# BaeHann/feature_level_style_transfer_for_TSC

Hardware: AMD Instinct MI355X
Metric: train-step samples/sec (univariate TS, len=512, batch=256) at 1/2/4/8 MI355X (higher is better)
Workload: dtype bf16x3

## Files before the change

### feature_level_style_transfer_for_tsc_amd/csrc/pointwise.hip

```cpp
#include "fst_common.h"

static thread_local char g_err[512] = "";
void fst_set_error(const char* fmt, ...) {
  va_list ap;
  va_start(ap, fmt);
  vsnprintf(g_err, sizeof(g_err), fmt, ap);
  va_end(ap);
}
extern "C" const char* fst_last_error(void) { return g_err; }

int fst_allow_full_lds(const void* fn, const char* who) {
  static const void* done[64];
  static int n_done = 0;
  for (int i = 0; i < n_done; ++i)
    if (done[i] == fn) return 0;
  hipError_t e = hipFuncSetAttribute(fn, hipFuncAttributeMaxDynamicSharedMemorySize, 160 * 1024);
  if (e != hipSuccess) {
    fst_set_error("%s: hipFuncSetAttribute: %s", who, hipGetErrorString(e));
    return (int)e;
  }
  if (n_done < 64) done[n_done++] = fn;
  return 0;
}
int fst_cu_count(void) {
  static int cached[16] = {0};
  int dev = 0;
  if (hipGetDevice(&dev) != hipSuccess || dev < 0 || dev >= 16) return 0;
  if (cached[dev] == 0) {
    int n = 0;
    if (hipDeviceGetAttribute(&n, hipDeviceAttributeMultiprocessorCount, dev) != hipSuccess) n = 0;
    cached[dev] = n > 0 ? n : -1;
  }
  return cached[dev] > 0 ? cached[dev] : 0;
}
extern "C" int fst_version(void) { return FST_ABI_VERSION; }

__device__ __forceinline__ float wave_sum(float v) {
#pragma unroll
  for (int o = 32; o > 0; o >>= 1) v += __shfl_down(v, o, 64);
  return v;
}

__device__ __forceinline__ void block_sum2(float& a, float& b) {
  __shared__ float sa[4], sb[4];
  a = wave_sum(a);
  b = wave_sum(b);
  const int lane = threadIdx.x & 63, wave = threadIdx.x >> 6;
  if (lane == 0) { sa[wave] = a; sb[wave] = b; }
  __syncthreads();
  if (threadIdx.x == 0) {
    a = sa[0] + sa[1] + sa[2] + sa[3];
    b = sb[0] + sb[1] + sb[2] + sb[3];
  }
  __syncthreads();
}

#define FST_REQUIRE_EXTENT(who, B, C, L, numel)                                                             \
  FST_REQUIRE((long long)(B) * (long long)(C) * (long long)(L) == (long long)(numel),                        \
              "%s: B*C*L = %d*%d*%d does not match the tensors' element count %lld", who, (int)(B), (int)(C), (int)(L), \
              (long long)(numel))


struct RowVec {
  int shift;
  int nv;
};
static inline bool vec_ok(int L, std::initializer_list<const void*> ptrs) {
  if (L % 4 != 0) return false;
  for (const void* q : ptrs)
    if (!fst_aligned16(q)) return false;
  return true;
}
static inline RowVec row_vec(int L) {
  RowVec v;
  v.nv = L / 4;
  v.shift = 0;
  while ((1 << v.shift) < v.nv && v.shift < 8) ++v.shift;
  return v;
}
static inline RowVec row_dword(int L, int shift) { return RowVec{shift, L}; }
constexpr int BN_DWORD_SHIFT = 8, ROW_SUM_DWORD_SHIFT = 6;

template <class V>
__device__ __forceinline__ RowVec row_geometry(RowVec rv, int dword_shift) {
  if (std::is_same_v<V, float>) rv.shift = dword_shift;
  return rv;
}
template <class V>
__device__ __forceinline__ int row_group(RowVec rv, int T) {
  const int r = threadIdx.x >> rv.shift;
  return std::is_same_v<V, float> ? r & ((T >> rv.shift) - 1) : r;
}

template <class Launch>
static inline void launch_rows(bool vec, int L, int dword_shift, Launch launch) {
  if (vec) launch(float4{}, row_vec(L));
  else launch(float{}, row_dword(L, dword_shift));
}

__device__ __forceinline__ float block_sum1024(float s) {
  __shared__ float sw[16];
  s = wave_sum(s);
  const int lane = threadIdx.x & 63, wave = threadIdx.x >> 6;
  if (lane == 0) sw[wave] = s;
  __syncthreads();
  float r = 0.f;
  if (threadIdx.x == 0) {
#pragma unroll
    for (int w = 0; w < 16; ++w) r += sw[w];
  }
  return r;
}

__device__ __forceinline__ void row_sum_add(float& s0, float& s1, const float4& v) {
  s0 += v.x + v.y;
  s1 += v.z + v.w;
}
__device__ __forceinline__ void row_sum_add(float& s0, float&, float v) { s0 += v; }

template <class V>
__global__ __launch_bounds__(1024) void row_sum_kernel(const float* x, long long x_bs, int B, int C, int L, float* out, RowVec rv) {
  rv = row_geometry<V>(rv, ROW_SUM_DWORD_SHIFT);
  const int c = blockIdx.x, r = row_group<V>(rv, 1024), t0 = threadIdx.x & ((1 << rv.shift) - 1), rpp = 1024 >> rv.shift;
  float s0 = 0.f, s1 = 0.f;
  for (int b = r; b < B; b += rpp) {
    const V* row = reinterpret_cast<const V*>(x + (long long)b * x_bs + (long long)c * L);
    for (int t = t0; t < rv.nv; t += 1 << rv.shift) {
      const V v = row[t];
      row_sum_add(s0, s1, v);
    }
  }
  const float s = block_sum1024(std::is_same_v<V, float> ? s0 : s0 + s1);
  if (threadIdx.x == 0) out[c] = s;
}

extern "C" int fst_row_sum(const float* x, int64_t x_bs, int B, int C, int L, float* out, void* stream) {
  FST_REQUIRE(x && out && B > 0 && C > 0 && L > 0, "fst_row_sum: bad arguments");
  FST_REQUIRE(B == 1 || x_bs >= (int64_t)C * L, "fst_row_sum: batch stride %lld < C*L = %lld", (long long)x_bs, (long long)C * L);
  launch_rows(vec_ok(L, {x}) && x_bs % 4 == 0, L, ROW_SUM_DWORD_SHIFT, [&](auto v, RowVec rv) {
    hipLaunchKernelGGL(row_sum_kernel<decltype(v)>, dim3(C), dim3(1024), 0, (hipStream_t)stream, x, (long long)x_bs, B, C, L, out, rv);
  });
  FST_LAUNCH_CHECK();
  return 0;
}

__device__ __forceinline__ void bn_moments_add(float& s1, float& s2, float v, float k) {
  const float d = v - k;
  s1 += d; s2 += d * d;
}
__device__ __forceinline__ void bn_moments_add(float& s1, float& s2, float4 v, float k) {
  const float dx = v.x - k, dy = v.y - k, dz = v.z - k, dw = v.w - k;
  s1 += (dx + dy) + (dz + dw);
  s2 += (dx * dx + dy * dy) + (dz * dz + dw * dw);
}

template <class V>
__global__ __launch_bounds__(256) void bn_stats_kernel(const float* y, int B, int C, int L, float* part, RowVec rv) {
  rv = row_geometry<V>(rv, BN_DWORD_SHIFT);
  const int c = blockIdx.x, r = row_group<V>(rv, 256), t0 = threadIdx.x & ((1 << rv.shift) - 1), rpp = 256 >> rv.shift;
  const float k = y[(long long)c * L];
  float s1 = 0.f, s2 = 0.f;
  for (int b = blockIdx.y + r * gridDim.y; b < B; b += rpp * gridDim.y) {
    const V* row = reinterpret_cast<const V*>(y + ((long long)b * C + c) * L);
    for (int t = t0; t < rv.nv; t += 1 << rv.shift) bn_moments_add(s1, s2, row[t], k);
  }
  block_sum2(s1, s2);
  if (threadIdx.x == 0) {
    const int rows = blockIdx.y < B ? (B - 1 - blockIdx.y) / gridDim.y + 1 : 0;
    float* o = part + ((long long)c * FST_BN_SLOTS + blockIdx.y) * 4;
    o[0] = (float)rows * (float)L; o[1] = k; o[2] = s1; o[3] = s2;
  }
}

extern "C" int fst_bn_stats(const float* y, int B, int C, int L, float* part, int64_t numel, void* stream) {
  FST_REQUIRE(y && part && B > 0 && C > 0 && L > 0, "fst_bn_stats: bad arguments");
  FST_REQUIRE_EXTENT("fst_bn_stats", B, C, L, numel);
  launch_rows(vec_ok(L, {y}), L, BN_DWORD_SHIFT, [&](auto v, RowVec rv) {
    hipLaunchKernelGGL(bn_stats_kernel<decltype(v)>, dim3(C, FST_BN_SLOTS), dim3(256), 0, (hipStream_t)stream, y, B, C, L, part, rv);
  });
  FST_LAUNCH_CHECK();
  return 0;
}

__global__ void bn_finalize_kernel(const float* part, int n_slots, const float* gamma, const float* beta, float* rmean,
                                   float* rvar, int train, int C, float eps, float momentum, float* stats) {
  const int c = blockIdx.x * blockDim.x + threadIdx.x;
  if (c >= C) return;
  float mean, var;
  if (train) {
    double n = 0.0, m = 0.0, m2 = 0.0;
    const float* q = part + (long long)c * n_slots * 4;
    for (int s = 0; s < n_slots; ++s) {
      const double nb = q[4 * s];
      if (nb <= 0.0) continue;
      const double s1 = q[4 * s + 2], s2 = q[4 * s + 3];
      const double mb = (double)q[4 * s + 1] + s1 / nb;
      double Mb = s2 - s1 * s1 / nb;
      if (Mb < 0.0) Mb = 0.0;
      const double nn = n + nb, d = mb - m;
      m += d * (nb / nn);
      m2 += Mb + d * d * (n * nb / nn);
      n = nn;
    }
    const double v = n > 0.0 ? m2 / n : 0.0;
    mean = (float)m;
    var = (float)v;
    const float unbiased = n > 1.0 ? (float)(m2 / (n - 1.0)) : var;
    rmean[c] = (1.f - momentum) * rmean[c] + momentum * mean;
    rvar[c] = (1.f - momentum) * rvar[c] + momentum * unbiased;
  } else {
    mean = rmean[c];
    var = rvar[c];
  }
  const float invstd = 1.0f / sqrtf(var + eps);
  const float scale = gamma[c] * invstd;
  stats[c] = mean;
  stats[C + c] = invstd;
  stats[2 * C + c] = scale;
  stats[3 * C + c] = beta[c] - mean * scale;
}

extern "C" int fst_bn_finalize(const float* part, int n_slots, const float* gamma, const float* beta, float* running_mean,
                               float* running_var, int train, int C, float eps, float momentum, float* stats, void* stream) {
  FST_REQUIRE(gamma && beta && running_mean && running_var && stats && C > 0, "fst_bn_finalize: bad arguments");
  FST_REQUIRE(!train || (part && n_slots > 0), "fst_bn_finalize: train mode needs the moment partials (n_slots=%d)", n_slots);
  hipLaunchKernelGGL(bn_finalize_kernel, dim3((C + 63) / 64), dim3(64), 0, (hipStream_t)stream, part, n_slots, gamma, beta,
                     running_mean, running_var, train, C, eps, momentum, stats);
  FST_LAUNCH_CHECK();
  return 0;
}

__device__ __forceinline__ float bn_pre(float y, float sc, float sh) { return __builtin_fmaf(y, sc, sh); }
__device__ __forceinline__ float bn_pre_join(float ya, float sca, float sha, float yb, float scb, float shb) {
#pragma clang fp contract(off)
  float v = bn_pre(ya, sca, sha);
  v += bn_pre(yb, scb, shb);
  return v;
}
__device__ __forceinline__ float4 bn_pre(float4 y, float sc, float sh) {
  return make_float4(bn_pre(y.x, sc, sh), bn_pre(y.y, sc, sh), bn_pre(y.z, sc, sh), bn_pre(y.w, sc, sh));
}
__device__ __forceinline__ float4 bn_pre_join(float4 ya, float sca, float sha, float4 yb, float scb, float shb) {
  return make_float4(bn_pre_join(ya.x, sca, sha, yb.x, scb, shb), bn_pre_join(ya.y, sca, sha, yb.y, scb, shb),
                     bn_pre_join(ya.z, sca, sha, yb.z, scb, shb), bn_pre_join(ya.w, sca, sha, yb.w, scb, shb));
}
__device__ __forceinline__ float bn_relu(float v) { return v < 0.f ? 0.f : v; }
__device__ __forceinline__ float4 bn_relu(float4 v) { return make_float4(bn_relu(v.x), bn_relu(v.y), bn_relu(v.z), bn_relu(v.w)); }

template <class V>
__global__ __launch_bounds__(256) void bn_apply_kernel(const float* y, const float* stats, const float* res,
                                                       const float* res_stats, float* out, int rows, int C, int L,
                                                       int relu, RowVec rv) {
  rv = row_geometry<V>(rv, BN_DWORD_SHIFT);
  const int r = row_group<V>(rv, 256), t0 = threadIdx.x & ((1 << rv.shift) - 1), rpp = 256 >> rv.shift;
  const int bc = blockIdx.x * rpp + r;
  if (bc >= rows) return;
  const int c = bc % C;
  const float sc = stats[2 * C + c], sh = stats[3 * C + c];
  float rsc = 1.f, rsh = 0.f;
  if (res && res_stats) { rsc = res_stats[2 * C + c]; rsh = res_stats[3 * C + c]; }
  const long long base = (long long)bc * rv.nv;
  const V* yv = reinterpret_cast<const V*>(y) + base;
  const V* qv = res ? reinterpret_cast<const V*>(res) + base : nullptr;
  V* ov = reinterpret_cast<V*>(out) + base;
  for (int t = t0; t < rv.nv; t += 1 << rv.shift) {
    V v = yv[t];
    v = qv ? bn_pre_join(v, sc, sh, qv[t], rsc, rsh) : bn_pre(v, sc, sh);
    if (relu) v = bn_relu(v);
    ov[t] = v;
  }
}

extern "C" int fst_bn_apply(const float* y, const float* stats, const float* res, const float* res_stats, float* out,
                            int B, int C, int L, int relu, int64_t numel, void* stream) {
  FST_REQUIRE(y && stats && out && B > 0 && C > 0 && L > 0, "fst_bn_apply: bad arguments");
  FST_REQUIRE_EXTENT("fst_bn_apply", B, C, L, numel);
  launch_rows(vec_ok(L, {y, res, out}), L, BN_DWORD_SHIFT, [&](auto v, RowVec rv) {
    const int rpp = 256 >> rv.shift;
    hipLaunchKernelGGL(bn_apply_kernel<decltype(v)>, dim3((B * C + rpp - 1) / rpp), dim3(256), 0, (hipStream_t)stream, y, stats,
                       res, res_stats, out, B * C, C, L, relu, rv);
  });
  FST_LAUNCH_CHECK();
  return 0;
}

__device__ __forceinline__ float bn_masked(float g, float o) { return o > 0.f ? g : 0.f; }
__device__ __forceinline__ float4 bn_masked(float4 g, float4 o) {
  g.x = bn_masked(g.x, o.x); g.y = bn_masked(g.y, o.y); g.z = bn_masked(g.z, o.z); g.w = bn_masked(g.w, o.w);
  return g;
}
__device__ __forceinline__ float bn_g(float g) { return g; }
__device__ __forceinline__ float bn_g(float4 g) {
#pragma clang fp contract(off)
  return (g.x + g.y) + (g.z + g.w);
}
__device__ __forceinline__ float bn_gx(float g, float y, float mean, float invstd) {
#pragma clang fp contract(off)
  return g * (y - mean) * invstd;
}
__device__ __forceinline__ float bn_gx(float4 g, float4 v, float mean, float invstd) {
#pragma clang fp contract(off)
  return (g.x * (v.x - mean) + g.y * (v.y - mean) + g.z * (v.z - mean) + g.w * (v.w - mean)) * invstd;
}
__device__ __forceinline__ float bn_dx_unscaled(float g, float y, float mean, float invstd, float m1, float m2) {
#pragma clang fp contract(off)
  const float xh = (y - mean) * invstd;
  return __builtin_fmaf(-xh, m2, g - m1);
}
__device__ __forceinline__ float4 bn_dx_unscaled(float4 g, float4 v, float mean, float invstd, float m1, float m2) {
  return make_float4(bn_dx_unscaled(g.x, v.x, mean, invstd, m1, m2), bn_dx_unscaled(g.y, v.y, mean, invstd, m1, m2),
                     bn_dx_unscaled(g.z, v.z, mean, invstd, m1, m2), bn_dx_unscaled(g.w, v.w, mean, invstd, m1, m2));
}
__device__ __forceinline__ float bn_dx(float scale, float u) {
#pragma clang fp contract(off)
  return scale * u;
}
__device__ __forceinline__ float4 bn_dx(float scale, float4 u) {
#pragma clang fp contract(off)
  return make_float4(scale * u.x, scale * u.y, scale * u.z, scale * u.w);
}
__device__ __forceinline__ float bn_row_sum_add(float rs, float scale, float u, float) { return __builtin_fmaf(scale, u, rs); }
__device__ __forceinline__ float bn_row_sum_add(float rs, float, float4, float4 d) {
#pragma clang fp contract(off)
  return rs + bn_g(d);
}

template <class V>
__global__ __launch_bounds__(256) void bn_bwd_reduce_kernel(const float* dy, const float* y, const float* out,
                                                            const float* stats, int B, int C, int L, int relu,
                                                            float* red, RowVec rv) {
#pragma clang fp contract(off)
  rv = row_geometry<V>(rv, BN_DWORD_SHIFT);
  const int c = blockIdx.x, r = row_group<V>(rv, 256), t0 = threadIdx.x & ((1 << rv.shift) - 1), rpp = 256 >> rv.shift;
  const float mean = stats[c], invstd = stats[C + c], sc = stats[2 * C + c], sh = stats[3 * C + c];
  float s1 = 0.f, s2 = 0.f;
  for (int b = blockIdx.y + r * gridDim.y; b < B; b += rpp * gridDim.y) {
    const long long base = ((long long)b * C + c) * rv.nv;
    const V* dyv = reinterpret_cast<const V*>(dy) + base;
    const V* yv = reinterpret_cast<const V*>(y) + base;
    const V* ov = reinterpret_cast<const V*>(out) + base;
    for (int t = t0; t < rv.nv; t += 1 << rv.shift) {
      V g = dyv[t];
      const V v = yv[t];
      if (relu) g = bn_masked(g, out ? ov[t] : bn_pre(v, sc, sh));
      s1 += bn_g(g);
      s2 += bn_gx(g, v, mean, invstd);
    }
  }
  block_sum2(s1, s2);
  if (threadIdx.x == 0) {
    red[(long long)c * FST_BN_SLOTS + blockIdx.y] = s1;
    red[((long long)C + c) * FST_BN_SLOTS + blockIdx.y] = s2;
  }
}

extern "C" int fst_bn_bwd_reduce(const float* dy, const float* y, const float* out, const float* stats, int B, int C,
                                 int L, int relu, float* red, int64_t numel, void* stream) {
  FST_REQUIRE(dy && y && stats && red && B > 0 && C > 0 && L > 0, "fst_bn_bwd_reduce: bad arguments");
  FST_REQUIRE_EXTENT("fst_bn_bwd_reduce", B, C, L, numel);
  if (!relu) out = nullptr;
  launch_rows(vec_ok(L, {dy, y, out}), L, BN_DWORD_SHIFT, [&](auto v, RowVec rv) {
    hipLaunchKernelGGL(bn_bwd_reduce_kernel<decltype(v)>, dim3(C, FST_BN_SLOTS), dim3(256), 0, (hipStream_t)stream, dy, y, out,
                       stats, B, C, L, relu, red, rv);
  });
  FST_LAUNCH_CHECK();
  return 0;
}

template <class V>
__global__ __launch_bounds__(256) void bn_bwd_reduce_join_kernel(const float* dy, const float* ya, const float* yb,
                                                                 const float* sa, const float* sb, int B, int C, int L,
                                                                 float* reda, float* redb, RowVec rv) {
#pragma clang fp contract(off)
  rv = row_geometry<V>(rv, BN_DWORD_SHIFT);
  const int c = blockIdx.x, r = row_group<V>(rv, 256), t0 = threadIdx.x & ((1 << rv.shift) - 1), rpp = 256 >> rv.shift;
  const float meana = sa[c], invstda = sa[C + c], sca = sa[2 * C + c], sha = sa[3 * C + c];
  const float meanb = sb[c], invstdb = sb[C + c], scb = sb[2 * C + c], shb = sb[3 * C + c];
  float s1 = 0.f, s2a = 0.f, s2b = 0.f, unused = 0.f;
  for (int b = blockIdx.y + r * gridDim.y; b < B; b += rpp * gridDim.y) {
    const long long base = ((long long)b * C + c) * rv.nv;
    const V* dyv = reinterpret_cast<const V*>(dy) + base;
    const V* yav = reinterpret_cast<const V*>(ya) + base;
    const V* ybv = reinterpret_cast<const V*>(yb) + base;
    for (int t = t0; t < rv.nv; t += 1 << rv.shift) {
      const V va = yav[t], vb = ybv[t];
      const V g = bn_masked(dyv[t], bn_pre_join(va, sca, sha, vb, scb, shb));
      s1 += bn_g(g);
      s2a += bn_gx(g, va, meana, invstda);
      s2b += bn_gx(g, vb, meanb, invstdb);
    }
  }
  block_sum2(s1, s2a);
  block_sum2(s2b, unused);
  if (threadIdx.x == 0) {
    reda[(long long)c * FST_BN_SLOTS + blockIdx.y] = s1;
    reda[((long long)C + c) * FST_BN_SLOTS + blockIdx.y] = s2a;
    redb[(long long)c * FST_BN_SLOTS + blockIdx.y] = s1;
    redb[((long long)C + c) * FST_BN_SLOTS + blockIdx.y] = s2b;
  }
}

extern "C" int fst_bn_bwd_reduce_join(const float* dy, const float* ya, const float* yb, const float* stats_a,
                                      const float* stats_b, int B, int C, int L, float* red_a, float* red_b, int64_t numel,
                                      void* stream) {
  FST_REQUIRE(dy && ya && yb && stats_a && stats_b && red_a && red_b && red_a != red_b && B > 0 && C > 0 && L > 0,
              "fst_bn_bwd_reduce_join: bad arguments");
  FST_REQUIRE_EXTENT("fst_bn_bwd_reduce_join", B, C, L, numel);
  launch_rows(vec_ok(L, {dy, ya, yb}), L, BN_DWORD_SHIFT, [&](auto v, RowVec rv) {
    hipLaunchKernelGGL(bn_bwd_reduce_join_kernel<decltype(v)>, dim3(C, FST_BN_SLOTS), dim3(256), 0, (hipStream_t)stream, dy, ya, yb,
                       stats_a, stats_b, B, C, L, red_a, red_b, rv);
  });
  FST_LAUNCH_CHECK();
  return 0;
}

__device__ __forceinline__ void bn_red_sums(const float* red, int n_slots, int C, int c, float& r1, float& r2) {
  r1 = 0.f; r2 = 0.f;
  for (int s = 0; s < n_slots; ++s) {
    r1 += red[(long long)c * n_slots + s];
    r2 += red[((long long)C + c) * n_slots + s];
  }
}

__device__ __forceinline__ void bn_row_sum_store(float rs, float* row_sums, int bc, bool live, int t0, RowVec rv, float* wsum) {
  const int w = rv.shift < 6 ? rv.shift : 6;
  for (int o = (1 << w) >> 1; o > 0; o >>= 1) rs += __shfl_xor(rs, o, 64);
  if (rv.shift <= 6) {
    if (live && t0 == 0) row_sums[bc] = rs;
  } else {
    if ((threadIdx.x & 63) == 0) wsum[threadIdx.x >> 6] = rs;
    __syncthreads();
    if (live && t0 == 0) {
// ... 496 lines not shown
```

### feature_level_style_transfer_for_tsc_amd/csrc/widgets.hip

```cpp
#include "fst_common.h"

#define NT_SELU_ALPHA 1.6732632423543772848170429916717f
#define NT_SELU_SCALE 1.0507009873554804934193349852946f

__global__ __launch_bounds__(256) void batch_sum_kernel(const float* x0, const float* x1, float* part, int B, long long N, int S) {
  const long long i4 = ((long long)blockIdx.x * 256 + threadIdx.x) * 4;
  if (i4 >= N) return;
  const int s = blockIdx.y;
  const float* x = blockIdx.z ? x1 : x0;
  const int b0 = (int)((long long)s * B / S), b1 = (int)((long long)(s + 1) * B / S);
  float4 acc = {0.f, 0.f, 0.f, 0.f};
  const float* q = x + (long long)b0 * N + i4;
#pragma unroll 8
  for (int b = b0; b < b1; ++b, q += N) {
    const float4 v = *reinterpret_cast<const float4*>(q);
    acc.x += v.x; acc.y += v.y; acc.z += v.z; acc.w += v.w;
  }
  *reinterpret_cast<float4*>(part + ((long long)blockIdx.z * S + s) * N + i4) = acc;
}

extern "C" int fst_batch_sum(const float* x0, const float* x1, float* part, int B, int64_t N, int S, void* stream) {
  FST_REQUIRE(x0 && part && B > 0 && N > 0 && N % 4 == 0 && S > 0 && S <= B, "fst_batch_sum: bad arguments (B=%d N=%lld S=%d; N %% 4 == 0, "
              "1 <= S <= B)", B, (long long)N, S);
  FST_REQUIRE(fst_aligned16(x0) && fst_aligned16(x1) && fst_aligned16(part), "fst_batch_sum: tensors must be 16-byte aligned");
  hipLaunchKernelGGL(batch_sum_kernel, dim3((unsigned)((N / 4 + 255) / 256), (unsigned)S, x1 ? 2 : 1), dim3(256), 0, (hipStream_t)stream,
                     x0, x1, part, B, (long long)N, S);
  FST_LAUNCH_CHECK();
  return 0;
}

struct NtFwdParams {
  const float* part;
  const float* r_t_dev;
  const float* r_s_dev;
  float r_t, r_s;
  float* avg_t;
  float* avg_s;
  const float* W;
  const float* bias;
  float* dist;
  float* pre;
  float* learned;
  int S, B, C, L;
};

__global__ __launch_bounds__(256) void noise_transfer_fwd_kernel(NtFwdParams p) {
  extern __shared__ float sd[];
  const int lx = threadIdx.x & 63, cg = threadIdx.x >> 6, l = blockIdx.x * 64 + lx;
  const int C = p.C, L = p.L, S = p.S;
  const long long N = (long long)C * L;
  const float rt = p.r_t_dev ? *p.r_t_dev : p.r_t, rs = p.r_s_dev ? *p.r_s_dev : p.r_s;
  const float fB = (float)p.B;
  if (l < L)
    for (int c = cg; c < C; c += 4) {
      const long long i = (long long)c * L + l;
      float st = 0.f, ss = 0.f;
      for (int s = 0; s < S; ++s) {
        st += p.part[(long long)s * N + i];
        ss += p.part[((long long)S + s) * N + i];
      }
      const float nt = p.avg_t[i] + rt * (st / fB), ns = p.avg_s[i] + rs * (ss / fB);
      p.avg_t[i] = nt;
      p.avg_s[i] = ns;
      const float d = nt - ns;
      p.dist[i] = d;
      sd[c * 64 + lx] = d;
    }
  __syncthreads();
  if (l < L)
    for (int o = cg; o < C; o += 4) {
      float acc = p.bias[o];
      const float* w = p.W + (long long)o * C;
      for (int c = 0; c < C; ++c) acc += w[c] * sd[c * 64 + lx];
      const long long i = (long long)o * L + l;
      p.pre[i] = acc;
      p.learned[i] = NT_SELU_SCALE * (acc > 0.f ? acc : NT_SELU_ALPHA * expm1f(acc));
    }
}

extern "C" int fst_noise_transfer_fwd(const float* part, int S, int B, const float* r_t_dev, const float* r_s_dev, float r_t, float r_s,
                                      float* avg_t, float* avg_s, const float* W, const float* bias, float* dist, float* pre,
                                      float* learned, int C, int L, void* stream) {
  FST_REQUIRE(part && avg_t && avg_s && W && bias && dist && pre && learned, "fst_noise_transfer_fwd: null operand");
  FST_REQUIRE(S > 0 && B > 0 && C > 0 && C <= 512 && L > 0, "fst_noise_transfer_fwd: bad shape S=%d B=%d C=%d L=%d (C <= 512)", S, B, C, L);
  NtFwdParams p = {part, r_t_dev, r_s_dev, r_t, r_s, avg_t, avg_s, W, bias, dist, pre, learned, S, B, C, L};
  const size_t lds = (size_t)C * 64 * sizeof(float);
  if (lds > 48 * 1024)
    if (int rc = fst_allow_full_lds((const void*)noise_transfer_fwd_kernel, "fst_noise_transfer_fwd")) return rc;
  hipLaunchKernelGGL(noise_transfer_fwd_kernel, dim3((unsigned)((L + 63) / 64)), dim3(256), lds, (hipStream_t)stream, p);
  FST_LAUNCH_CHECK();
  return 0;
}

__global__ __launch_bounds__(256) void bcast_add_kernel(float* out, const float* x, const float* v, long long N4, long long total4) {
  for (long long j = (long long)blockIdx.x * 256 + threadIdx.x; j < total4; j += (long long)gridDim.x * 256) {
    const float4 a = reinterpret_cast<const float4*>(x)[j], b = reinterpret_cast<const float4*>(v)[j % N4];
    reinterpret_cast<float4*>(out)[j] = {a.x + b.x, a.y + b.y, a.z + b.z, a.w + b.w};
  }
}

extern "C" int fst_bcast_add(float* out, const float* x, const float* v, int B, int64_t N, void* stream) {
  FST_REQUIRE(out && x && v && B > 0 && N > 0 && N % 4 == 0, "fst_bcast_add: bad arguments (B=%d N=%lld, N %% 4 == 0)", B, (long long)N);
  FST_REQUIRE(fst_aligned16(out) && fst_aligned16(x) && fst_aligned16(v), "fst_bcast_add: tensors must be 16-byte aligned");
  const long long total4 = (long long)B * N / 4;
  long long blocks = (total4 + 255) / 256;
  if (blocks > 8192) blocks = 8192;
  hipLaunchKernelGGL(bcast_add_kernel, dim3((unsigned)blocks), dim3(256), 0, (hipStream_t)stream, out, x, v, (long long)(N / 4), total4);
  FST_LAUNCH_CHECK();
  return 0;
}

struct NtBwdParams {
  const float* part;
  const float* pre;
  const float* W;
  float* dpre;
  float* dd;
  int S, C, L;
};

__global__ __launch_bounds__(256) void noise_transfer_bwd_kernel(NtBwdParams p) {
  extern __shared__ float sd[];
  const int lx = threadIdx.x & 63, cg = threadIdx.x >> 6, l = blockIdx.x * 64 + lx;
  const int C = p.C, L = p.L, S = p.S;
  const long long N = (long long)C * L;
  if (l < L)
    for (int o = cg; o < C; o += 4) {
      const long long i = (long long)o * L + l;
      float G = 0.f;
      for (int s = 0; s < S; ++s) G += p.part[(long long)s * N + i];
      const float x = p.pre[i];
      const float dp = G * NT_SELU_SCALE * (x > 0.f ? 1.0f : NT_SELU_ALPHA * expf(x));
      p.dpre[i] = dp;
      sd[o * 64 + lx] = dp;
    }
  __syncthreads();
  if (l < L)
    for (int c = cg; c < C; c += 4) {
      float acc = 0.f;
      for (int o = 0; o < C; ++o) acc += p.W[(long long)o * C + c] * sd[o * 64 + lx];
      p.dd[(long long)c * L + l] = acc;
    }
}

extern "C" int fst_noise_transfer_bwd(const float* part, int S, const float* pre, const float* W, float* dpre, float* dd, int C, int L,
                                      void* stream) {
  FST_REQUIRE(part && pre && W && dpre && dd, "fst_noise_transfer_bwd: null operand");
  FST_REQUIRE(S > 0 && C > 0 && C <= 512 && L > 0, "fst_noise_transfer_bwd: bad shape S=%d C=%d L=%d (C <= 512)", S, C, L);
  NtBwdParams p = {part, pre, W, dpre, dd, S, C, L};
  const size_t lds = (size_t)C * 64 * sizeof(float);
  if (lds > 48 * 1024)
    if (int rc = fst_allow_full_lds((const void*)noise_transfer_bwd_kernel, "fst_noise_transfer_bwd")) return rc;
  hipLaunchKernelGGL(noise_transfer_bwd_kernel, dim3((unsigned)((L + 63) / 64)), dim3(256), lds, (hipStream_t)stream, p);
  FST_LAUNCH_CHECK();
  return 0;
}

__global__ __launch_bounds__(256) void noise_transfer_dw_kernel(const float* dpre, const float* dist, float* dW, float* dbias, int C, int L) {
  const int o = blockIdx.x, lane = threadIdx.x & 63, w = threadIdx.x >> 6;
  const float* dp = dpre + (long long)o * L;
  for (int c = w; c <= C; c += 4) {
    float acc = 0.f;
    if (c < C) {
      const float* x = dist + (long long)c * L;
      for (int l = lane; l < L; l += 64) acc += dp[l] * x[l];
    } else {
      for (int l = lane; l < L; l += 64) acc += dp[l];
    }
#pragma unroll
    for (int m = 32; m >= 1; m >>= 1) acc += __shfl_xor(acc, m, 64);
    if (lane == 0) {
      if (c < C) dW[(long long)o * C + c] = acc;
      else dbias[o] = acc;
    }
  }
}

extern "C" int fst_noise_transfer_dw(const float* dpre, const float* dist, float* dW, float* dbias, int C, int L, void* stream) {
  FST_REQUIRE(dpre && dist && dW && dbias && C > 0 && L > 0, "fst_noise_transfer_dw: bad arguments");
  hipLaunchKernelGGL(noise_transfer_dw_kernel, dim3((unsigned)C), dim3(256), 0, (hipStream_t)stream, dpre, dist, dW, dbias, C, L);
  FST_LAUNCH_CHECK();
  return 0;
}

__global__ __launch_bounds__(256) void noise_transfer_bwd_apply_kernel(const float* g, const float* dd, const float* r_t_dev,
                                                                       const float* r_s_dev, float r_t, float r_s, int B, float* dz_t,
                                                                       float* dz_s, long long N4, long long total4) {
  const float fB = (float)B;
  const float kt = (r_t_dev ? *r_t_dev : r_t) / fB, ks = (r_s_dev ? *r_s_dev : r_s) / fB;
  for (long long j = (long long)blockIdx.x * 256 + threadIdx.x; j < total4; j += (long long)gridDim.x * 256) {
    const float4 d = reinterpret_cast<const float4*>(dd)[j % N4];
    if (dz_t) reinterpret_cast<float4*>(dz_t)[j] = {kt * d.x, kt * d.y, kt * d.z, kt * d.w};
    if (dz_s) {
      const float4 a = reinterpret_cast<const float4*>(g)[j];
      reinterpret_cast<float4*>(dz_s)[j] = {a.x - ks * d.x, a.y - ks * d.y, a.z - ks * d.z, a.w - ks * d.w};
    }
  }
}

extern "C" int fst_noise_transfer_bwd_apply(const float* g, const float* dd, const float* r_t_dev, const float* r_s_dev, float r_t,
                                            float r_s, int B, float* dz_t, float* dz_s, int64_t N, void* stream) {
  FST_REQUIRE(g && dd && (dz_t || dz_s) && B > 0 && N > 0 && N % 4 == 0, "fst_noise_transfer_bwd_apply: bad arguments (B=%d N=%lld)", B,
              (long long)N);
  FST_REQUIRE(fst_aligned16(g) && fst_aligned16(dd) && fst_aligned16(dz_t) && fst_aligned16(dz_s), "fst_noise_transfer_bwd_apply: tensors must be 16-byte aligned");
  const long long total4 = (long long)B * N / 4;
  long long blocks = (total4 + 255) / 256;
  if (blocks > 8192) blocks = 8192;
  hipLaunchKernelGGL(noise_transfer_bwd_apply_kernel, dim3((unsigned)blocks), dim3(256), 0, (hipStream_t)stream, g, dd, r_t_dev, r_s_dev,
                     r_t, r_s, B, dz_t, dz_s, (long long)(N / 4), total4);
  FST_LAUNCH_CHECK();
  return 0;
}

__global__ __launch_bounds__(256) void relu_bwd_kernel(const float* dy, const float* y, float* out, long long n4, long long n) {
  for (long long j = (long long)blockIdx.x * 256 + threadIdx.x; j < n4; j += (long long)gridDim.x * 256) {
    const float4 g = reinterpret_cast<const float4*>(dy)[j], v = reinterpret_cast<const float4*>(y)[j];
    reinterpret_cast<float4*>(out)[j] = {v.x > 0.f ? g.x : 0.f, v.y > 0.f ? g.y : 0.f, v.z > 0.f ? g.z : 0.f, v.w > 0.f ? g.w : 0.f};
  }
  if (blockIdx.x == 0)
    for (long long i = 4 * n4 + threadIdx.x; i < n; i += 256) out[i] = y[i] > 0.f ? dy[i] : 0.f;
}

extern "C" int fst_relu_bwd(const float* dy, const float* y, float* out, int64_t n, void* stream) {
  FST_REQUIRE(dy && y && out && n > 0, "fst_relu_bwd: bad arguments");
  FST_REQUIRE(fst_aligned16(dy) && fst_aligned16(y) && fst_aligned16(out), "fst_relu_bwd: tensors must be 16-byte aligned");
  long long blocks = (n / 4 + 255) / 256;
  if (blocks > 8192) blocks = 8192;
  if (blocks < 1) blocks = 1;
  hipLaunchKernelGGL(relu_bwd_kernel, dim3((unsigned)blocks), dim3(256), 0, (hipStream_t)stream, dy, y, out, (long long)(n / 4), (long long)n);
  FST_LAUNCH_CHECK();
  return 0;
}
```

Before: 3702.

## Split noise-transfer kernels into state and conv passes with wider grids

The fused noise-transfer forward and backward kernels, which staged a C×64 tile in LDS and looped over channels per block, are each split into two launches. An elementwise pass handles state and derivative updates, and a 2D-grid pass does the channel-mixing matmul reading global memory directly. The dW kernel now spreads channels across a second grid dimension, and row_sum gains a fast path for few channels with short rows. The aim is more parallelism and fewer large-LDS blocks when L is small, at the cost of extra launches and repeated global reads of dist and dpre.

New measurement: 3722 (median of 6 runs). About the same (+0.5%).

```diff
diff --git a/feature_level_style_transfer_for_tsc_amd/csrc/pointwise.hip b/feature_level_style_transfer_for_tsc_amd/csrc/pointwise.hip
--- a/feature_level_style_transfer_for_tsc_amd/csrc/pointwise.hip
+++ b/feature_level_style_transfer_for_tsc_amd/csrc/pointwise.hip
@@ -118,16 +118,26 @@
 }
 __device__ __forceinline__ void row_sum_add(float& s0, float&, float v) { s0 += v; }
 
+constexpr int ROW_SUM_FEW_ROWS = 64;
+
 template <class V>
 __global__ __launch_bounds__(1024) void row_sum_kernel(const float* x, long long x_bs, int B, int C, int L, float* out, RowVec rv) {
   rv = row_geometry<V>(rv, ROW_SUM_DWORD_SHIFT);
   const int c = blockIdx.x, r = row_group<V>(rv, 1024), t0 = threadIdx.x & ((1 << rv.shift) - 1), rpp = 1024 >> rv.shift;
   float s0 = 0.f, s1 = 0.f;
-  for (int b = r; b < B; b += rpp) {
-    const V* row = reinterpret_cast<const V*>(x + (long long)b * x_bs + (long long)c * L);
-    for (int t = t0; t < rv.nv; t += 1 << rv.shift) {
-      const V v = row[t];
-      row_sum_add(s0, s1, v);
+  if (C <= ROW_SUM_FEW_ROWS && rv.nv <= 1 << rv.shift) {
+    if (t0 < rv.nv) {
+      const float* p = x + (long long)c * L;
+#pragma unroll 8
+      for (int b = r; b < B; b += rpp) row_sum_add(s0, s1, reinterpret_cast<const V*>(p + (long long)b * x_bs)[t0]);
+    }
+  } else {
+    for (int b = r; b < B; b += rpp) {
+      const V* row = reinterpret_cast<const V*>(x + (long long)b * x_bs + (long long)c * L);
+      for (int t = t0; t < rv.nv; t += 1 << rv.shift) {
+        const V v = row[t];
+        row_sum_add(s0, s1, v);
+      }
     }
   }
   const float s = block_sum1024(std::is_same_v<V, float> ? s0 : s0 + s1);
diff --git a/feature_level_style_transfer_for_tsc_amd/csrc/widgets.hip b/feature_level_style_transfer_for_tsc_amd/csrc/widgets.hip
--- a/feature_level_style_transfer_for_tsc_amd/csrc/widgets.hip
+++ b/feature_level_style_transfer_for_tsc_amd/csrc/widgets.hip
@@ -44,38 +44,37 @@
   int S, B, C, L;
 };
 
-__global__ __launch_bounds__(256) void noise_transfer_fwd_kernel(NtFwdParams p) {
-  extern __shared__ float sd[];
-  const int lx = threadIdx.x & 63, cg = threadIdx.x >> 6, l = blockIdx.x * 64 + lx;
-  const int C = p.C, L = p.L, S = p.S;
-  const long long N = (long long)C * L;
+__global__ __launch_bounds__(256) void noise_transfer_state_kernel(NtFwdParams p) {
+  const int S = p.S;
+  const long long N = (long long)p.C * p.L, i = (long long)blockIdx.x * 256 + threadIdx.x;
+  if (i >= N) return;
   const float rt = p.r_t_dev ? *p.r_t_dev : p.r_t, rs = p.r_s_dev ? *p.r_s_dev : p.r_s;
   const float fB = (float)p.B;
-  if (l < L)
-    for (int c = cg; c < C; c += 4) {
-      const long long i = (long long)c * L + l;
-      float st = 0.f, ss = 0.f;
-      for (int s = 0; s < S; ++s) {
-        st += p.part[(long long)s * N + i];
-        ss += p.part[((long long)S + s) * N + i];
-      }
-      const float nt = p.avg_t[i] + rt * (st / fB), ns = p.avg_s[i] + rs * (ss / fB);
-      p.avg_t[i] = nt;
-      p.avg_s[i] = ns;
-      const float d = nt - ns;
-      p.dist[i] = d;
-      sd[c * 64 + lx] = d;
-    }
-  __syncthreads();
-  if (l < L)
-    for (int o = cg; o < C; o += 4) {
-      float acc = p.bias[o];
-      const float* w = p.W + (long long)o * C;
-      for (int c = 0; c < C; ++c) acc += w[c] * sd[c * 64 + lx];
-      const long long i = (long long)o * L + l;
-      p.pre[i] = acc;
-      p.learned[i] = NT_SELU_SCALE * (acc > 0.f ? acc : NT_SELU_ALPHA * expm1f(acc));
-    }
+  float st = 0.f, ss = 0.f;
+#pragma unroll 8
+  for (int s = 0; s < S; ++s) {
+    st += p.part[(long long)s * N + i];
+    ss += p.part[((long long)S + s) * N + i];
+  }
+  const float nt = p.avg_t[i] + rt * (st / fB), ns = p.avg_s[i] + rs * (ss / fB);
+  p.avg_t[i] = nt;
+  p.avg_s[i] = ns;
+  const float d = nt - ns;
+  p.dist[i] = d;
+}
+
+__global__ __launch_bounds__(256) void noise_transfer_conv_kernel(NtFwdParams p) {
+  const int C = p.C, L = p.L;
+  const int l = blockIdx.x * 64 + (threadIdx.x & 63), o = __builtin_amdgcn_readfirstlane(blockIdx.y * 4 + (threadIdx.x >> 6));
+  if (l >= L || o >= C) return;
+  float acc = p.bias[o];
+  const float* w = p.W + (long long)o * C;
+  const float* d = p.dist + l;
+#pragma unroll 8
+  for (int c = 0; c < C; ++c) acc += w[c] * d[(long long)c * L];
+  const long long i = (long long)o * L + l;
+  p.pre[i] = acc;
+  p.learned[i] = NT_SELU_SCALE * (acc > 0.f ? acc : NT_SELU_ALPHA * expm1f(acc));
 }
 
 extern "C" int fst_noise_transfer_fwd(const float* part, int S, int B, const float* r_t_dev, const float* r_s_dev, float r_t, float r_s,
@@ -84,10 +83,10 @@
   FST_REQUIRE(part && avg_t && avg_s && W && bias && dist && pre && learned, "fst_noise_transfer_fwd: null operand");
   FST_REQUIRE(S > 0 && B > 0 && C > 0 && C <= 512 && L > 0, "fst_noise_transfer_fwd: bad shape S=%d B=%d C=%d L=%d (C <= 512)", S, B, C, L);
   NtFwdParams p = {part, r_t_dev, r_s_dev, r_t, r_s, avg_t, avg_s, W, bias, dist, pre, learned, S, B, C, L};
-  const size_t lds = (size_t)C * 64 * sizeof(float);
-  if (lds > 48 * 1024)
-    if (int rc = fst_allow_full_lds((const void*)noise_transfer_fwd_kernel, "fst_noise_transfer_fwd")) return rc;
-  hipLaunchKernelGGL(noise_transfer_fwd_kernel, dim3((unsigned)((L + 63) / 64)), dim3(256), lds, (hipStream_t)stream, p);
+  const long long N = (long long)C * L;
+  hipLaunchKernelGGL(noise_transfer_state_kernel, dim3((unsigned)((N + 255) / 256)), dim3(256), 0, (hipStream_t)stream, p);
+  hipLaunchKernelGGL(noise_transfer_conv_kernel, dim3((unsigned)((L + 63) / 64), (unsigned)((C + 3) / 4)), dim3(256), 0,
+                     (hipStream_t)stream, p);
   FST_LAUNCH_CHECK();
   return 0;
 }
@@ -119,28 +118,28 @@
   int S, C, L;
 };
 
-__global__ __launch_bounds__(256) void noise_transfer_bwd_kernel(NtBwdParams p) {
-  extern __shared__ float sd[];
-  const int lx = threadIdx.x & 63, cg = threadIdx.x >> 6, l = blockIdx.x * 64 + lx;
-  const int C = p.C, L = p.L, S = p.S;
-  const long long N = (long long)C * L;
-  if (l < L)
-    for (int o = cg; o < C; o += 4) {
-      const long long i = (long long)o * L + l;
-      float G = 0.f;
-      for (int s = 0; s < S; ++s) G += p.part[(long long)s * N + i];
-      const float x = p.pre[i];
-      const float dp = G * NT_SELU_SCALE * (x > 0.f ? 1.0f : NT_SELU_ALPHA * expf(x));
-      p.dpre[i] = dp;
-      sd[o * 64 + lx] = dp;
-    }
-  __syncthreads();
-  if (l < L)
-    for (int c = cg; c < C; c += 4) {
-      float acc = 0.f;
-      for (int o = 0; o < C; ++o) acc += p.W[(long long)o * C + c] * sd[o * 64 + lx];
-      p.dd[(long long)c * L + l] = acc;
-    }
+__global__ __launch_bounds__(256) void noise_transfer_dpre_kernel(NtBwdParams p) {
+  const int S = p.S;
+  const long long N = (long long)p.C * p.L, i = (long long)blockIdx.x * 256 + threadIdx.x;
+  if (i >= N) return;
+  float G = 0.f;
+#pragma unroll 8
+  for (int s = 0; s < S; ++s) G += p.part[(long long)s * N + i];
+  const float x = p.pre[i];
+  const float dp = G * NT_SELU_SCALE * (x > 0.f ? 1.0f : NT_SELU_ALPHA * expf(x));
+  p.dpre[i] = dp;
+}
+
+__global__ __launch_bounds__(256) void noise_transfer_dd_kernel(NtBwdParams p) {
+  const int C = p.C, L = p.L;
+  const int l = blockIdx.x * 64 + (threadIdx.x & 63), c = __builtin_amdgcn_readfirstlane(blockIdx.y * 4 + (threadIdx.x >> 6));
+  if (l >= L || c >= C) return;
+  float acc = 0.f;
+  const float* w = p.W + c;
+  const float* d = p.dpre + l;
+#pragma unroll 8
+  for (int o = 0; o < C; ++o) acc += w[(long long)o * C] * d[(long long)o * L];
+  p.dd[(long long)c * L + l] = acc;
 }
 
 extern "C" int fst_noise_transfer_bwd(const float* part, int S, const float* pre, const float* W, float* dpre, float* dd, int C, int L,
@@ -148,37 +147,38 @@
   FST_REQUIRE(part && pre && W && dpre && dd, "fst_noise_transfer_bwd: null operand");
   FST_REQUIRE(S > 0 && C > 0 && C <= 512 && L > 0, "fst_noise_transfer_bwd: bad shape S=%d C=%d L=%d (C <= 512)", S, C, L);
   NtBwdParams p = {part, pre, W, dpre, dd, S, C, L};
-  const size_t lds = (size_t)C * 64 * sizeof(float);
-  if (lds > 48 * 1024)
-    if (int rc = fst_allow_full_lds((const void*)noise_transfer_bwd_kernel, "fst_noise_transfer_bwd")) return rc;
-  hipLaunchKernelGGL(noise_transfer_bwd_kernel, dim3((unsigned)((L + 63) / 64)), dim3(256), lds, (hipStream_t)stream, p);
+  const long long N = (long long)C * L;
+  hipLaunchKernelGGL(noise_transfer_dpre_kernel, dim3((unsigned)((N + 255) / 256)), dim3(256), 0, (hipStream_t)stream, p);
+  hipLaunchKernelGGL(noise_transfer_dd_kernel, dim3((unsigned)((L + 63) / 64), (unsigned)((C + 3) / 4)), dim3(256), 0,
+                     (hipStream_t)stream, p);
   FST_LAUNCH_CHECK();
   return 0;
 }
 
 __global__ __launch_bounds__(256) void noise_transfer_dw_kernel(const float* dpre, const float* dist, float* dW, float* dbias, int C, int L) {
-  const int o = blockIdx.x, lane = threadIdx.x & 63, w = threadIdx.x >> 6;
+  const int o = blockIdx.x, lane = threadIdx.x & 63, c = __builtin_amdgcn_readfirstlane(blockIdx.y * 4 + (threadIdx.x >> 6));
+  if (c > C) return;
   const float* dp = dpre + (long long)o * L;
-  for (int c = w; c <= C; c += 4) {
-    float acc = 0.f;
-    if (c < C) {
-      const float* x = dist + (long long)c * L;
-      for (int l = lane; l < L; l += 64) acc += dp[l] * x[l];
-    } else {
-      for (int l = lane; l < L; l += 64) acc += dp[l];
-    }
+  float acc = 0.f;
+  if (c < C) {
+    const float* x = dist + (long long)c * L;
+    for (int l = lane; l < L; l += 64) acc += dp[l] * x[l];
+  } else {
+    for (int l = lane; l < L; l += 64) acc += dp[l];
+  }
 #pragma unroll
-    for (int m = 32; m >= 1; m >>= 1) acc += __shfl_xor(acc, m, 64);
-    if (lane == 0) {
-      if (c < C) dW[(long long)o * C + c] = acc;
-      else dbias[o] = acc;
-    }
+  for (int m = 32; m >= 1; m >>= 1) acc += __shfl_xor(acc, m, 64);
+  if (lane == 0) {
+    if (c < C) dW[(long long)o * C + c] = acc;
+    else dbias[o] = acc;
   }
 }
 
 extern "C" int fst_noise_transfer_dw(const float* dpre, const float* dist, float* dW, float* dbias, int C, int L, void* stream) {
   FST_REQUIRE(dpre && dist && dW && dbias && C > 0 && L > 0, "fst_noise_transfer_dw: bad arguments");
-  hipLaunchKernelGGL(noise_transfer_dw_kernel, dim3((unsigned)C), dim3(256), 0, (hipStream_t)stream, dpre, dist, dW, dbias, C, L);
+  FST_REQUIRE(C <= 4 * 65535 - 1, "fst_noise_transfer_dw: C = %d is more than the grid covers", C);
+  hipLaunchKernelGGL(noise_transfer_dw_kernel, dim3((unsigned)C, (unsigned)((C + 1 + 3) / 4)), dim3(256), 0, (hipStream_t)stream, dpre,
+                     dist, dW, dbias, C, L);
   FST_LAUNCH_CHECK();
   return 0;
 }
```
